# wangqiaoli/geometric_mapping

Hardware: AMD Instinct MI355X
Metric: points/sec full segment+fit, 1M-pt synthetic tunnel frame (higher is better)
Workload: dtype f32; 1 GPU; 1000000-pt synthetic tunnel frame (R=2 m, L=12 m, sigma=0.01), rows resident in HBM; k_regime=fixed-k (~256 neighbours), mode=frames, frames_in_flight=4, GPU_MAX_HW_QUEUES=4, ransac_model=cylinder, H=1024, tau=0.03 (extension), parallelism=framesx1

## Files before the change

geometric_mapping_amd/csrc/k_normals.hip:

```cpp
#include <stdlib.h>
#include <string.h>

#include "gm_internal.hpp"

namespace gm {

typedef float v2f __attribute__((ext_vector_type(2)));

__device__ __forceinline__ v2f pk_mul_rn(v2f a, v2f b)
{
    v2f r;
    r.x = __fmul_rn(a.x, b.x);
    r.y = __fmul_rn(a.y, b.y);
    return r;
}
__device__ __forceinline__ v2f pk_add_rn(v2f a, v2f b)
{
    v2f r;
    r.x = __fadd_rn(a.x, b.x);
    r.y = __fadd_rn(a.y, b.y);
    return r;
}

__device__ __forceinline__ v2f pk_within(v2f d2, v2f neg_big, v2f r2_big)
// ... 391 lines not shown
    uint64_t remaining = __ballot(vox_ok);
    while (remaining) {
        const int leader = (int)__builtin_ctzll(remaining);
        const uint32_t k = __shfl(vkey, leader, kWave);
        const bool mine = vox_ok && vkey == k;
        const uint64_t same = __ballot(mine);
        const unsigned long long ax = wave_total_u64(mine ? fx : 0ull);
        const unsigned long long ay = wave_total_u64(mine ? fy : 0ull);
        const unsigned long long az = wave_total_u64(mine ? fz : 0ull);
        if (lane == leader) {
            VoxCell *cell = vox_table + k;
            atomicAdd(&cell->sx, ax);
            atomicAdd(&cell->sy, ay);
            atomicAdd(&cell->sz, az);
            atomicAdd(&cell->cnt, (uint32_t)__popcll(same));
        }
        remaining &= ~same;
    }
}

struct NormalsArgs {
    const float4 *__restrict__ spts4;
    const uint32_t *__restrict__ skeys;
    const uint2 *__restrict__ tiles;
    DevCounters *__restrict__ ctr;
    GridParams g;
    uint32_t tiles_cap;
    uint32_t tile_seg;
    const uint2 *__restrict__ row_bounds;
    float4 *__restrict__ normals4;
    int32_t *__restrict__ counts;
    VoxDense vd;
    VoxCell *__restrict__ vox_table;
};

constexpr int kValuWaveLdsBytes = 3 * (kWinCap + kWinPad) * 4 + 10 * kWave * 8;
__device__ __forceinline__ void normals_tile_valu(const NormalsArgs &A, unsigned char *lds, const uint2 tile)
{
    const float4 *__restrict__ spts4 = A.spts4;
    const uint32_t *__restrict__ skeys = A.skeys;
    DevCounters *__restrict__ ctr = A.ctr;
    const GridParams &g = A.g;
    const uint2 *__restrict__ row_bounds = A.row_bounds;
    float4 *__restrict__ normals4 = A.normals4;
    int32_t *__restrict__ counts = A.counts;
    const VoxDense &vd = A.vd;
    VoxCell *__restrict__ vox_table = A.vox_table;
    (void)ctr;
    typedef float WinT[3][kWinCap + kWinPad];
    typedef double TotT[10][kWave];
    WinT *win = reinterpret_cast<WinT *>(lds);
    TotT *tot = reinterpret_cast<TotT *>(lds + sizeof(WinT));
    const int lane = lane_id();
    const int w = 0;
    const uint32_t n = ctr->n_cropped;
    {
        const uint32_t qs = tile.x, qn = tile.y & 0xFFu;
#ifdef GM_NORMALS_TIMELINE
        const unsigned long long stat_t0 = wall_clock64();
#endif

        const int ql = lane;
        const bool active = (uint32_t)ql < qn;
        const uint32_t qidx = qs + (active ? (uint32_t)ql : qn - 1u);
        const float4 q = spts4[qidx];
        const uint32_t kl = skeys[qidx];
// ... 434 lines not shown
constexpr int kMdChunk = GM_MDCHUNK;
constexpr int kMdSlots = kMdChunk + 24;
constexpr int kMdOctets = kMdSlots / 8;
constexpr int kMdOctetWords = 33 * 4;
constexpr int kMdWaveLdsBytes = (kMdOctets * kMdOctetWords + 16) * 4;

constexpr int kRowX[3] = {1, 4, 8}, kRowY[3] = {2, 5, 9}, kRowZ[3] = {3, 6, 10}, kRowQ[3] = {11, 7, 12};
constexpr int kRowProd0 = 13;
__device__ __forceinline__ uint32_t md_window_of_base(int b)
{
    return b < 3 ? 0u : ((b == 3 || b == 8) ? 4u : (b == 9 ? 8u : (b == 10 ? 12u : 0u)));
}
__device__ __forceinline__ void md_split3(float a, uint32_t out[3])
{
    const uint32_t ah = __float_as_uint(a) & 0xFFFF0000u;
    const float ra = a - __uint_as_float(ah);
    const uint32_t am = __float_as_uint(ra) & 0xFFFF0000u;
    const float sa = ra - __uint_as_float(am);
    out[0] = ah >> 16; out[1] = am >> 16; out[2] = __float_as_uint(sa) >> 16;
}
__device__ __forceinline__ s4 md_tr_read(const unsigned char *p)
{
    return __builtin_amdgcn_ds_read_tr16_b64_v4i16((__attribute__((address_space(3))) s4 *)p);
}

#ifndef GM_NORMALS_PREFETCH
#define GM_NORMALS_PREFETCH 1
#endif
#ifdef GM_NORMALS_TIMELINE
__device__ unsigned long long gm_tl_buf[3 * 65536];
#endif
#ifdef GM_NORMALS_PHASES
__device__ unsigned long long gm_phase_ticks[16];
#define GM_PH_STAMP(var) const unsigned long long var = __builtin_amdgcn_s_memtime()
#define GM_PH_ADD(slot, expr) do { ph_acc[slot] += (uint32_t)(expr); } while (0)
#else
#define GM_PH_STAMP(var) do {} while (0)
#define GM_PH_ADD(slot, expr) do {} while (0)
#endif

template <bool FINE>
__device__ __forceinline__ void normals_tile_mxd(const NormalsArgs &A, unsigned char *lds, const uint2 tile, uint32_t min_candidates,
                                                 unsigned long long stat_entry = 0ull)
{
    const float4 *__restrict__ spts4 = A.spts4;
    const uint32_t *__restrict__ skeys = A.skeys;
    DevCounters *__restrict__ ctr = A.ctr;
    const GridParams &g = A.g;
    const uint2 *__restrict__ row_bounds = A.row_bounds;
    float4 *__restrict__ normals4 = A.normals4;
    int32_t *__restrict__ counts = A.counts;
    const VoxDense &vd = A.vd;
    VoxCell *__restrict__ vox_table = A.vox_table;
    (void)ctr;
    uint32_t *feat = reinterpret_cast<uint32_t *>(lds);
    int lane = lane_id();
    asm volatile("" : "+v"(lane));
    const uint32_t n = ctr->n_cropped;
    const int qsel = lane & 31, half = lane >> 5;
    const int tq = (lane & 15) >> 2, tp = lane & 3, tr0 = 16 * ((lane >> 4) & 1);
    const uint32_t tr_off = md_window_of_base(8 * half + tq) * 16u +
                            (uint32_t)((tr0 + 4 * tp) >> 3) * (uint32_t)(kMdOctetWords * 4) + (uint32_t)((tr0 + 4 * tp) & 7) * 2u;
    const uint32_t mom_off = (uint32_t)qsel * 16u + 8u * (uint32_t)half;
    {
        const uint32_t qs = tile.x, qn = tile.y & 0xFFu, tile_row = tile.y >> 8;
#ifdef GM_NORMALS_TIMELINE
        const unsigned long long stat_t0 = wall_clock64();
#else
        const unsigned long long stat_t0 = 0ull;
#endif
#ifdef GM_NORMALS_PHASES
        uint32_t ph_acc[8] = {0, 0, 0, 0, 0, 0, 0, 0};
#endif
        GM_PH_STAMP(ph_t0);
        const bool active = (uint32_t)lane < qn;
        const uint32_t qidx = qs + (active ? (uint32_t)lane : qn - 1u);
        const float4 q = spts4[qidx];
        const uint32_t kl = skeys[qidx];
        const uint32_t row = tile_row;
        const int cy = (int)(row % (uint32_t)g.ny), cz = (int)(row / (uint32_t)g.ny);
        const int gD = FINE ? g.D : 1;
        const int side = 2 * gD + 1, nrows_all = side * side;
        int nrows = 0;
        struct LaneRow { int gg, reach; uint32_t nrow; bool ok; uint2 rb; };
        auto lane_row = [&](int row0) -> LaneRow {
            nrows = nrows_all - row0 < 32 ? nrows_all - row0 : 32;
            const int k = FINE ? lane : (lane >> 1);
            const int r = row0 + (k >> 1);
            const int a = (r % side) - gD, b = (r / side) - gD;
            const int yy = cy + a, zz = cz + b;
            LaneRow R;
            R.gg = k & 1;
            R.reach = (k >> 1) < nrows ? (FINE ? (int)g.reach[a < 0 ? -a : a][b < 0 ? -b : b] : g.xreach) : 0;
            R.ok = R.reach > 0 && yy >= 0 && yy < g.ny && zz >= 0 && zz < g.nz;
            R.nrow = R.ok ? (uint32_t)(zz * g.ny + yy) : 0u;
            R.rb = R.ok ? row_bounds[R.nrow] : make_uint2(0u, 0u);
            return R;
        };
        const LaneRow lr0 = lane_row(0);
        const int fxl = (int)(kl - row * (uint32_t)g.nx);
        if (__ballot(active && q.x >= vd.own_lo && q.x < vd.own_hi) == 0) {
            if (active) {
                const float nanv = __builtin_nanf("");
                normals4[__float_as_uint(q.w)] = make_float4(nanv, nanv, nanv, nanv);
                if (counts) counts[__float_as_uint(q.w)] = 0;
            }
            return;
        }
        uint32_t sb = 0, se = 0;
        auto win_begin = [&](int r, int gg) -> uint32_t {
            return FINE ? __builtin_amdgcn_readlane(sb, r * kMxGroups + gg) : __builtin_amdgcn_readlane(sb, 2 * (r * kMxGroups + gg));
        };
        auto win_end = [&](int r, int gg) -> uint32_t {
            return FINE ? __builtin_amdgcn_readlane(se, r * kMxGroups + gg) : __builtin_amdgcn_readlane(sb, 2 * (r * kMxGroups + gg) + 1);
        };
        auto find_windows = [&](const LaneRow &R) {
            sb = 0; se = 0;
            const int gg = R.gg, reach = R.reach;
            const int lo_fx = __shfl(fxl, gg * kMxGroupLanes, kWave);
            const int hi_fx = __shfl(fxl, gg * kMxGroupLanes + kMxGroupLanes - 1, kWave);
            uint32_t key_b = 0, key_e = 0, lo1 = 0, hi1 = 0, row_key0 = 0;
            if (R.ok) {
                const uint32_t rbk = R.nrow * (uint32_t)g.nx;
                const int xa = lo_fx > reach ? lo_fx - reach : 0;
                const int xb = hi_fx + reach < g.nx - 1 ? hi_fx + reach : g.nx - 1;
                key_b = rbk + (uint32_t)xa; key_e = rbk + (uint32_t)xb + 1u;
                lo1 = R.rb.x; hi1 = R.rb.y; row_key0 = rbk;
            }
            if (FINE) {
                uint32_t lo2 = lo1, hi2 = hi1;
                while (lo1 < hi1 || lo2 < hi2) {
                    const uint32_t m1 = (lo1 + hi1) >> 1, m2 = (lo2 + hi2) >> 1;
                    const uint32_t k1 = skeys[m1 < n ? m1 : n - 1u], k2 = skeys[m2 < n ? m2 : n - 1u];
                    if (lo1 < hi1) { if (k1 < key_b) lo1 = m1 + 1u; else hi1 = m1; }
                    if (lo2 < hi2) { if (k2 < key_e) lo2 = m2 + 1u; else hi2 = m2; }
                }
                sb = lo1; se = lo2;
            } else {
                const uint32_t key = (lane & 1) ? key_e : key_b;
#ifndef GM_NORMALS_NO_GUIDED_PROBE
                constexpr uint32_t kGuide = 64;
                if (hi1 - lo1 > 8u * kGuide) {
                    const uint32_t xq = key - row_key0;
                    const uint32_t gpos = lo1 + (uint32_t)((float)xq * (float)(hi1 - lo1) / (float)g.nx);
                    const uint32_t pa0 = gpos > lo1 + kGuide ? gpos - kGuide : lo1;
                    const uint32_t pb0 = gpos + kGuide < hi1 ? gpos + kGuide : hi1 - 1u;
                    const uint32_t ka0 = skeys[pa0], kb0 = skeys[pb0];
                    if (ka0 < key) lo1 = pa0 + 1u; else hi1 = pa0;
                    if (pb0 >= lo1 && pb0 < hi1) { if (kb0 < key) lo1 = pb0 + 1u; else hi1 = pb0; }
                }
#endif
                while (lo1 < hi1) {
                    const uint32_t m1 = (lo1 + hi1) >> 1;
                    if (skeys[m1] < key) lo1 = m1 + 1u; else hi1 = m1;
                }
                sb = lo1;
            }
        };
        find_windows(lr0);
        GM_PH_STAMP(ph_t1);
        GM_PH_ADD(0, ph_t1 - ph_t0);
        bool thin = false;
        if (!FINE) {
            uint32_t wl = 0;
#pragma unroll
            for (int r = 0; r < 9; ++r)
                wl += win_end(r, 0) - win_begin(r, 0);
            thin = wl < min_candidates;
        }
        const int mid = (int)(qn >> 1);
        const float inv_snap = 1.0f / g.snap;
        const float ox = rintf(__uint_as_float(__builtin_amdgcn_readlane(__float_as_uint(q.x), mid)) * inv_snap) * g.snap,
                    oy = rintf(__uint_as_float(__builtin_amdgcn_readlane(__float_as_uint(q.y), mid)) * inv_snap) * g.snap,
                    oz = rintf(__uint_as_float(__builtin_amdgcn_readlane(__float_as_uint(q.z), mid)) * inv_snap) * g.snap;
#ifdef GM_MD_DEBUG
        const float band = g.band;
#endif
        const int ngroups = qn > (uint32_t)kMxGroupLanes ? 2 : 1;
        f32x16 acc[kMxGroups];

#pragma unroll
        for (int gi = 0; gi < kMxGroups; ++gi)
#pragma unroll
            for (int k = 0; k < 16; ++k) acc[gi][k] = 0.f;

        bf16x8 qb[kMxGroups][2];
        float gq[kMxGroups][3];
#pragma unroll
        for (int gi = 0; gi < kMxGroups; ++gi) {
            gq[gi][0] = __shfl(q.x, gi * kMxGroupLanes + qsel, kWave);
            gq[gi][1] = __shfl(q.y, gi * kMxGroupLanes + qsel, kWave);
            gq[gi][2] = __shfl(q.z, gi * kMxGroupLanes + qsel, kWave);
            const float vx = gq[gi][0] - ox, vy = gq[gi][1] - oy, vz = gq[gi][2] - oz;
            const float vv = __fadd_rn(__fadd_rn(__fmul_rn(vx, vx), __fmul_rn(vy, vy)), __fmul_rn(vz, vz));
            uint32_t sv[3], sx[3], sy[3], sz[3];
            const float S = g.dscale;
            md_split3(__fsub_rn(g.r2, vv) * S, sv); md_split3(2.0f * S * vx, sx); md_split3(2.0f * S * vy, sy); md_split3(2.0f * S * vz, sz);
            const uint32_t one = __float_as_uint(-S) >> 16;
            const uint32_t lo0[8] = {sv[0], sv[1], sv[2], sx[0], sx[0], sx[1], sx[2], sy[0]};
            const uint32_t lo1[8] = {sy[0], sy[1], sy[2], sz[0], sz[0], sz[1], sz[2], one};
            const uint32_t hi0[8] = {sx[1], sx[0], one, 0u, sy[1], sy[0], 0u, 0u};
            const uint32_t hi1[8] = {sz[1], sz[0], 0u, 0u, 0u, one, 0u, 0u};
            union { bf16x8 v; uint32_t u[4]; } f0, f1;
#pragma unroll
            for (int j = 0; j < 4; ++j) {
                f0.u[j] = half ? (hi0[2 * j] | (hi0[2 * j + 1] << 16)) : (lo0[2 * j] | (lo0[2 * j + 1] << 16));
                f1.u[j] = half ? (hi1[2 * j] | (hi1[2 * j + 1] << 16)) : (lo1[2 * j] | (lo1[2 * j + 1] << 16));
            }
            qb[gi][0] = f0.v; qb[gi][1] = f1.v;
        }
        auto row_begin = [&](int r) -> uint32_t { return win_begin(r, 0); };
        auto row_end = [&](int r) -> uint32_t { return win_end(r, ngroups - 1); };
        if (thin) {
#if defined(GM_NORMALS_STATS) && !defined(GM_MD_DEBUG)
            if (lane == 0) atomicAdd(&ctr->pad[4], 1u);
#endif
            double tm[10] = {0, 0, 0, 0, 0, 0, 0, 0, 0, 0};
            for (int r = 0; r < 9; ++r) {
                const uint32_t e = row_end(r);
                for (uint32_t i = row_begin(r); i < e; ++i) {
                    const float4 c = spts4[i];
                    const float dx = c.x - q.x, dy = c.y - q.y, dz = c.z - q.z;
                    const float d2 = __fadd_rn(__fadd_rn(__fmul_rn(dx, dx), __fmul_rn(dy, dy)), __fmul_rn(dz, dz));
                    if (d2 < g.r2) {
                        const double ex = dx, ey = dy, ez = dz;
                        tm[0] += 1.0; tm[1] += ex; tm[2] += ey; tm[3] += ez;
                        tm[4] += ex * ex; tm[5] += ex * ey; tm[6] += ex * ez; tm[7] += ey * ey; tm[8] += ey * ez; tm[9] += ez * ez;
                    }
                }
            }
            const bool vox_ok = emit_normal(active, q, tm, vd, normals4, counts, qn, stat_t0);
            if (vd.enabled) voxel_sums(vox_ok, q, vd, vox_table);
            return;
        }
        uint32_t gs = 0, stream_total = 0, nxt_c = 0;
        const int endl = 2 * (ngroups - 1) + 1;
        if (!FINE) {
            const int rl = lane & ~3;
            const uint32_t rb = __shfl(sb, rl, kWave), re = __shfl(sb, rl + endl, kWave);
            const bool rowlane = lane < 36;
            const uint32_t len = rowlane ? re - rb : 0u;
            const uint32_t padded = (len + 7u) & ~7u;
            uint32_t incl = padded;
            incl += (uint32_t)__builtin_amdgcn_update_dpp(0, (int)incl, 0x114 , 0xF, 0xF, true);
            incl += (uint32_t)__builtin_amdgcn_update_dpp(0, (int)incl, 0x118 , 0xF, 0xF, true);
            incl += (uint32_t)__builtin_amdgcn_update_dpp(0, (int)incl, 0x142 , 0xA, 0xF, false);
            incl += (uint32_t)__builtin_amdgcn_update_dpp(0, (int)incl, 0x143 , 0xC, 0xF, false);
            const uint32_t srow = incl - padded;
            const uint32_t s_next = __shfl(incl, 4 * (lane - 40), kWave);
            const uint32_t off_r = __shfl(rb - srow, 4 * (lane - 50), kWave);
            gs = rowlane ? srow + (sb - rb) : ((lane >= 40 && lane < 49) ? s_next : ((lane >= 50 && lane < 59) ? off_r : 0u));
            stream_total = __builtin_amdgcn_readlane(gs, 48);
        }
        GM_PH_STAMP(ph_t2);
        GM_PH_ADD(1, ph_t2 - ph_t1);
        static_assert(kMdChunk == 2 * kWave, "one slot pair per lane and chunk");
        constexpr int kMdPieces = 4;
        int cur_r = 0, row0 = 0;
        uint32_t cur_c = row_begin(0);
        uint32_t n_lo[kMxGroups], n_hi[kMxGroups], n_slots = 0;
        float4 pa = make_float4(0.f, 0.f, 0.f, 0.f), pb = pa;
        uint32_t pidx = qs, pv = 0;
        auto assemble_stream = [&]() {
            n_slots = 0; pv = 0; pidx = qs;
#pragma unroll
            for (int gi = 0; gi < kMxGroups; ++gi) { n_lo[gi] = 0xFFFFFFFFu; n_hi[gi] = 0u; }
// ... 5 lines not shown
            uint32_t r = 0;
#pragma unroll
            for (int k = 0; k < 9; ++k) r += sl0 >= (uint32_t)__builtin_amdgcn_readlane(gs, 40 + k) ? 1u : 0u;
            r = r > 8u ? 8u : r;
            const uint32_t off = __shfl(gs, 50 + (int)r, kWave), lim = __shfl(gs, 4 * (int)r + endl, kWave);
            const bool v0 = sl0 < lim, v1 = sl0 + 1u < lim;
            pidx = v0 ? sl0 + off : qs;
            pv = v0 ? (v1 ? 3u : 1u) : 0u;
            const uint32_t other = __shfl_xor(gs, 1, kWave);
            const uint32_t cb = gs > c0 ? gs : c0, ce = other < c1 ? other : c1;
            const uint64_t m = __ballot((lane & 1) == 0 && lane < 36 && ce > cb);
            const uint32_t cb8 = (cb & ~7u) - c0, ce0 = ce - c0;
#pragma unroll
            for (int gi = 0; gi < kMxGroups; ++gi) {
                if (gi >= ngroups) break;
                const uint64_t mg = m & (gi ? 0x444444444ull : 0x111111111ull);
                if (mg) {
                    n_lo[gi] = __builtin_amdgcn_readlane(cb8, (int)__builtin_ctzll(mg));
                    n_hi[gi] = __builtin_amdgcn_readlane(ce0, 63 - (int)__builtin_clzll(mg));
                }
            }
            pa = spts4[pidx];
            pb = spts4[pidx + (pv >> 1)];
        };
        auto assemble_walk = [&]() {
            n_slots = 0; pv = 0; pidx = qs;
#pragma unroll
            for (int gi = 0; gi < kMxGroups; ++gi) { n_lo[gi] = 0xFFFFFFFFu; n_hi[gi] = 0u; }
            int pieces = 0;
            for (;;) {
                if (cur_r >= nrows) {
                    if (!FINE || row0 + 32 >= nrows_all) break;
                    row0 += 32;
                    find_windows(lane_row(row0));
                    cur_r = 0; cur_c = row_begin(0);
                    continue;
                }
                const uint32_t e = row_end(cur_r);
                if (cur_c >= e) {
                    ++cur_r;
                    if (cur_r < nrows) cur_c = row_begin(cur_r);
                    continue;
                }
                const uint32_t len = e - cur_c, room = (uint32_t)kMdChunk - n_slots;
                const uint32_t take = len < room ? len : room;
#pragma unroll
                for (int gi = 0; gi < kMxGroups; ++gi) {
                    if (gi >= ngroups) break;
                    const uint32_t mb = win_begin(cur_r, gi), me = win_end(cur_r, gi);
                    uint32_t ob = mb > cur_c ? mb - cur_c : 0u, oe = me > cur_c ? me - cur_c : 0u;
                    if (ob > take) ob = take;
                    if (oe > take) oe = take;
                    if (oe > ob) {
                        const uint32_t l = n_slots + (ob & ~7u), h = n_slots + oe;
                        n_lo[gi] = l < n_lo[gi] ? l : n_lo[gi];
                        n_hi[gi] = h > n_hi[gi] ? h : n_hi[gi];
                    }
                }
                {
                    const uint32_t i = 2u * (uint32_t)lane;
                    const bool in = i >= n_slots && i < n_slots + take;
                    pidx = in ? cur_c + (i - n_slots) : pidx;
                    pv = in ? (i + 1u < n_slots + take ? 3u : 1u) : pv;
                }
                n_slots += (take + 7u) & ~7u;
                cur_c += take;
                ++pieces;
// ... 137 lines not shown
                    if (__ballot(amin < g.dband)) {
                        uint32_t gqi = (uint32_t)(gi * kMxGroupLanes + qsel);
                        gqi = qs + (gqi < qn ? gqi : qn - 1u);
                        asm volatile("" : "+v"(gqi));
                        const float4 gqv = spts4[gqi];
#pragma unroll
                        for (int k = 0; k < 16; ++k) {
                            const uint32_t rk = (uint32_t)((k & 3) + 8 * (k >> 2) + 4 * half);
                            const bool need = fabsf(d1[k]) < g.dband;
                            if (__ballot(need)) {
                                if (need) {
                                    const float4 c = spts4[feat[((p + rk) >> 3) * (uint32_t)kMdOctetWords + 31u * 4u + ((p + rk) & 7u)]];
                                    const float dx = c.x - gqv.x, dy = c.y - gqv.y, dz = c.z - gqv.z;
                                    const float d2 = __fadd_rn(__fadd_rn(__fmul_rn(dx, dx), __fmul_rn(dy, dy)), __fmul_rn(dz, dz));
                                    const uint32_t wk = (d2 < g.r2 ? 1u : 0u) * 0x3F80u;
                                    pw[k >> 1] = (k & 1) ? ((pw[k >> 1] & 0x0000FFFFu) | (wk << 16)) : ((pw[k >> 1] & 0xFFFF0000u) | wk);
                                }
                            }
                        }
                    }
                    union { bf16x8 v; uint32_t u[4]; } b0, b1;
#pragma unroll
                    for (int k = 0; k < 4; ++k) { b0.u[k] = pw[k]; b1.u[k] = pw[4 + k]; }
                    acc[gi] = __builtin_amdgcn_mfma_f32_32x32x16_bf16(m0.v, b0.v, acc[gi], 0, 0, 0);
                    acc[gi] = __builtin_amdgcn_mfma_f32_32x32x16_bf16(m1.v, b1.v, acc[gi], 0, 0, 0);
                }
            }
#if !GM_NORMALS_PREFETCH
            assemble();
#endif
            GM_PH_STAMP(ph_c3);
            GM_PH_ADD(4, ph_c3 - ph_c2);
        }
        GM_PH_STAMP(ph_t3);
        int lane_e = lane_id();
        asm volatile("" : "+v"(lane_e));
        const int half_e = lane_e >> 5;
        const bool active_e = (uint32_t)lane_e < qn;
        float own[16], got[16];
#pragma unroll
        for (int k = 0; k < 16; ++k) {
            own[k] = half_e ? acc[1][k] : acc[0][k];
            const float snd = half_e ? acc[0][k] : acc[1][k];
            got[k] = __shfl_xor(snd, 32, kWave);
        }
        auto frow = [&](int rr) -> double {
            const int k = 4 * (rr >> 3) + (rr & 3), hh = (rr >> 2) & 1;
            return (double)((hh == half_e) ? own[k] : got[k]);
        };
        double mom[10];
        mom[0] = frow(0);
        mom[1] = (frow(kRowX[0]) + frow(kRowX[1])) + frow(kRowX[2]);
        mom[2] = (frow(kRowY[0]) + frow(kRowY[1])) + frow(kRowY[2]);
        mom[3] = (frow(kRowZ[0]) + frow(kRowZ[1])) + frow(kRowZ[2]);
#pragma unroll
        for (int m = 0; m < 6; ++m) mom[4 + m] = (frow(kRowProd0 + 3 * m) + frow(kRowProd0 + 3 * m + 1)) + frow(kRowProd0 + 3 * m + 2);

        uint32_t qidx_e = qs + (active_e ? (uint32_t)lane_e : qn - 1u);
        asm volatile("" : "+v"(qidx_e));
        const float4 qe = spts4[qidx_e];
        const bool vox_ok = emit_normal(active_e, qe, mom, vd, normals4, counts, qn, stat_t0, stat_entry);
        if (vd.enabled) voxel_sums(vox_ok, qe, vd, vox_table);
        GM_PH_STAMP(ph_t4);
        GM_PH_ADD(5, ph_t4 - ph_t3);
        GM_PH_ADD(6, ph_t4 - ph_t0);
        GM_PH_ADD(7, 1);
#ifdef GM_NORMALS_PHASES
        if (lane < 8) {
            uint32_t v = 0;
#pragma unroll
            for (int k = 0; k < 8; ++k) v = lane == k ? ph_acc[k] : v;
            atomicAdd(&gm_phase_ticks[lane], (unsigned long long)v);
        }
#endif
    }
}

constexpr int kWaveLdsBytes = (kMxWaveLdsBytes + 15) / 16 * 16;

struct TileList {
    uint32_t n;
    uint32_t pre[kTileClasses];
};
__device__ __forceinline__ TileList tile_list(const NormalsArgs &A)
{
    TileList L;
    uint32_t run = 0;
#pragma unroll
    for (int c = 0; c < kTileClasses; ++c) {
        uint32_t k = A.ctr->n_tiles_c[c][0];
        const uint32_t cap = c + 1 < kTileClasses ? A.tile_seg : A.tiles_cap;
        if (k > cap) k = cap;
        L.pre[c] = run;
        run += k;
    }
    L.n = run;
    return L;
}
__device__ __forceinline__ uint2 tile_at(const NormalsArgs &A, const TileList &L, uint32_t v)
{
    uint32_t c = 0, first = 0;
#pragma unroll
    for (int k = 1; k < kTileClasses; ++k)
        if (v >= L.pre[k]) { c = (uint32_t)k; first = L.pre[k]; }
    return A.tiles[(size_t)c * A.tile_seg + (v - first)];
}

__device__ __forceinline__ uint32_t normals_wave_id(const NormalsArgs &A, uint32_t ntiles)
{
    uint32_t vblock = blockIdx.x;
    const uint32_t nblk = (ntiles + kNrWaves - 1) / kNrWaves;
    if (gridDim.x >= nblk && A.vd.xcd_chunk) {
        if (blockIdx.x >= nblk) return 0xFFFFFFFFu;
        const uint32_t cb = A.vd.xcd_chunk, full = nblk / (8u * cb) * (8u * cb);
        if (blockIdx.x < full) {
            const uint32_t xcd = blockIdx.x % 8u, slot = blockIdx.x / 8u;
            vblock = ((slot / cb) * 8u + xcd) * cb + slot % cb;
        }
    }
    return (uint32_t)__builtin_amdgcn_readfirstlane((int)(vblock * kNrWaves + threadIdx.x / kWave));
}

__global__ __launch_bounds__(kNrThreads, GM_MX_WAVES) void k_normals_m(NormalsArgs A, uint32_t mx_min_candidates)
{
    __shared__ __attribute__((aligned(16))) unsigned char lds[kNrWaves][kWaveLdsBytes];
    const TileList L = tile_list(A);
    const uint32_t ntiles = L.n;
    const uint32_t wave_id = normals_wave_id(A, ntiles), n_waves = gridDim.x * kNrWaves;
    for (uint32_t t = wave_id; t < ntiles; t += n_waves)
        normals_tile_mx(A, lds[threadIdx.x / kWave], tile_at(A, L, t), mx_min_candidates);
}

template <bool FINE>
__global__ __launch_bounds__(kNrThreads, GM_MX_WAVES) void k_normals(NormalsArgs A, uint32_t mx_min_candidates)
{
    __shared__ __attribute__((aligned(16))) unsigned char lds[kNrWaves][(kMdWaveLdsBytes + 15) / 16 * 16];
#ifdef GM_NORMALS_TIMELINE
    unsigned long long stat_entry;
    asm volatile("s_memrealtime %0\n\ts_waitcnt lgkmcnt(0)" : "=s"(stat_entry) : : "memory");
#else
    const unsigned long long stat_entry = 0ull;
#endif
    const TileList L = tile_list(A);
    const uint32_t ntiles = L.n;
    const uint32_t wave_id = normals_wave_id(A, ntiles), n_waves = gridDim.x * kNrWaves;
    if (wave_id >= ntiles) return;
    const int wv = __builtin_amdgcn_readfirstlane((int)(threadIdx.x / kWave));
    {
        uint4 *z = reinterpret_cast<uint4 *>(lds[wv]);
        for (int i = lane_id(); i < kMdWaveLdsBytes / 16; i += kWave) z[i] = make_uint4(0u, 0u, 0u, 0u);
    }
#ifdef GM_NORMALS_TIMELINE
    const uint2 tile_tl = tile_at(A, L, wave_id);
    unsigned long long stat_tile;
    asm volatile("s_memrealtime %0\n\ts_waitcnt lgkmcnt(0)" : "=s"(stat_tile) : "v"(tile_tl.x) : "memory");
    normals_tile_mxd<FINE>(A, lds[wv], tile_tl, mx_min_candidates, stat_entry);
    if (wave_id < 65536u && lane_id() == 0) {
        gm_tl_buf[3 * wave_id + 0] = stat_entry;
        gm_tl_buf[3 * wave_id + 1] = stat_tile;
        gm_tl_buf[3 * wave_id + 2] = (unsigned long long)wall_clock64();
    }
#else
    normals_tile_mxd<FINE>(A, lds[wv], tile_at(A, L, wave_id), mx_min_candidates, stat_entry);
#endif
#ifndef GM_NORMALS_NO_LOOP
    if (ntiles > n_waves && wave_id != 0xFFFFFFFFu)
        for (uint32_t t = wave_id + n_waves; t < ntiles; t += n_waves)
            normals_tile_mxd<FINE>(A, lds[wv], tile_at(A, L, t), mx_min_candidates);
#endif
}

__global__ __launch_bounds__(kNrThreads) void k_normals_valu(NormalsArgs A)
{
    __shared__ __attribute__((aligned(16))) unsigned char lds[kNrWaves][(kValuWaveLdsBytes + 15) / 16 * 16];
    const TileList L = tile_list(A);
    const uint32_t ntiles = L.n;
    const uint32_t wave_id = normals_wave_id(A, ntiles), n_waves = gridDim.x * kNrWaves;
    for (uint32_t t = wave_id; t < ntiles; t += n_waves) normals_tile_valu(A, lds[threadIdx.x / kWave], tile_at(A, L, t));
}

int cell_key_bits(const GridParams &g)
{
    const uint64_t ncell = (uint64_t)g.nx * g.ny * g.nz;
    int bits = 1;
    while ((1ull << bits) < ncell) ++bits;
    return bits;
}

static double inv_below(uint32_t d) { return nextafter(1.0 / (double)(d ? d : 1u), 0.0); }

uint32_t max_tiles(uint32_t n_cap, const GridParams &g)
{
    const uint64_t span = (uint64_t)kTileSpan * (uint64_t)(g.xreach - 1);
    const uint64_t groups = (uint64_t)g.ny * (uint64_t)g.nz * ((uint64_t)g.nx / (span + 1) + 1);
    const uint64_t extra = (groups < n_cap ? groups : n_cap) + n_cap / kTileQ;
    return (uint32_t)(n_cap / kTileQ + extra + 1);
}

void launch_grid_and_normals(const GridParams &g, const VoxDense &vd, Slot &sl, uint32_t n_cap, bool keep_counts,
                             bool scratch_cleared, hipStream_t s)
{
    if (n_cap == 0) return;
    const int where = launch_radix_sort(sl.keys_a, sl.vals_a, sl.keys_b, sl.vals_b, &sl.ctr->n_cropped, n_cap, cell_key_bits(g),
                                        sl, scratch_cleared, s, sl.crop4, sl.spts4);
    uint32_t *skeys = where ? sl.keys_b : sl.keys_a;
    sl.skeys = skeys;
    if (!scratch_cleared) hipMemsetAsync(sl.row_bounds, 0, sizeof(uint2) * (size_t)g.ny * (size_t)g.nz, s);
    {
        ScanState st = next_scan(sl);
        st.status = sl.tile_rec;
        st.ticket = sl.sort.ticket + 1;
        static const char *to = getenv("GM_TILE_ORDER");
        const uint32_t single_class = to ? (to[0] == 'p' ? 1u : 0u) : (sl.pipelined ? 1u : 0u);
        hipLaunchKernelGGL(k_rows_and_tiles, dim3(tile_cutter_blocks(n_cap)), dim3(kTbThreads), 0, s, (const uint32_t *)skeys, sl.ctr,
                           (uint32_t)g.nx, (uint32_t)(kTileSpan * (g.xreach - 1)), inv_below((uint32_t)g.nx),
                           inv_below((uint32_t)(kTileSpan * (g.xreach - 1)) + 1u), sl.row_bounds, (uint32_t)g.ny * (uint32_t)g.nz, sl.tiles,
                           sl.tiles_cap, sl.tile_seg, st, single_class);
    }
    const uint32_t mt = max_tiles(n_cap, g);
    uint32_t nb = (mt + kNrWaves - 1) / kNrWaves;
    {
        const uint32_t usual = (n_cap / 32u + kNrWaves) / kNrWaves;
        if (nb > usual) nb = usual < 64u ? 64u : usual;
    }
    {
        static const char *e = getenv("GM_NORMALS_BLOCKS");
        const uint32_t cap = e ? (uint32_t)atoi(e) : 65536u;
        if (nb > cap) nb = cap;
    }
    static const char *xc = getenv("GM_NORMALS_XCD");
    VoxDense vdx = vd;
    vdx.xcd_chunk = xc ? (uint32_t)atoi(xc) : 32u;
    NormalsArgs na;
    na.spts4 = sl.spts4; na.skeys = skeys; na.tiles = sl.tiles; na.ctr = sl.ctr; na.g = g; na.tiles_cap = sl.tiles_cap; na.tile_seg = sl.tile_seg;
    na.row_bounds = sl.row_bounds; na.normals4 = sl.normals4; na.counts = keep_counts ? sl.counts : (int32_t *)nullptr;
    na.vd = vdx; na.vox_table = sl.vox_table;
    static const char *impl = getenv("GM_NORMALS_IMPL");
    const uint32_t mx_min = !impl ? (uint32_t)kMxMinCandidates : (impl[0] == 'v' ? 0xFFFFFFFFu : (impl[0] == 'm' ? 0u : (uint32_t)kMxMinCandidates));
    if (!sl.capturing) hipEventRecord(sl.ev_k0, s);
    const bool dist_on_mx = !(impl && strchr(impl, '0'));
    if (mx_min == 0xFFFFFFFFu) hipLaunchKernelGGL(k_normals_valu, dim3(nb), dim3(kNrThreads), 0, s, na);
    else if (dist_on_mx) {
        if (g.D > 1) hipLaunchKernelGGL(k_normals<true>, dim3(nb), dim3(kNrThreads), 0, s, na, mx_min);
        else hipLaunchKernelGGL(k_normals<false>, dim3(nb), dim3(kNrThreads), 0, s, na, mx_min);
    }
    else hipLaunchKernelGGL(k_normals_m, dim3(nb), dim3(kNrThreads), 0, s, na, mx_min);
    if (!sl.capturing) hipEventRecord(sl.ev_k1, s);
}

}

#ifdef GM_NORMALS_STATS
extern "C" int gm_debug_counters(gm_ctx *ctx, uint32_t slot, uint32_t *out)
{
    hipDeviceSynchronize();
    gm::DevCounters c;
    const int rc = (int)hipMemcpy(&c, ctx->slots[slot].ctr, sizeof(c), hipMemcpyDeviceToHost);
    memcpy(out, &c, 18 * sizeof(uint32_t));
    out[2] = 0;
    for (int k = 0; k < gm::kTileListClasses; ++k) out[2] += c.n_tiles_c[k][0];
    return rc;
}
#endif

#ifdef GM_NORMALS_TIMELINE
extern "C" int gm_debug_timeline(unsigned long long *out, uint32_t n)
{
    hipDeviceSynchronize();
    if (n > 65536u) n = 65536u;
    return (int)hipMemcpyFromSymbol(out, HIP_SYMBOL(gm::gm_tl_buf), sizeof(unsigned long long) * 3 * (size_t)n);
}
#endif

// ... 19 lines not shown
```

Baseline: 5.303 billion points/s.

## Process tile pairs per wave, overlapping next tile's head loads with epilogue

Each normals wave now handles two consecutive tiles. It issues the second tile's query, key and row-bound loads and its guided-probe search loads while the first tile's epilogue solve and voxel sums run. When both tiles share a grid row, the first tile's window start seeds the second tile's binary search to shrink its range. The block count is halved, which reduces parallelism and occupancy and adds register pressure from holding two tile states. Pairing is on by default for the non-fine MX path and can be disabled with an environment variable.

New measurement: 5.180 billion points/s. 2.3% lower.

```diff
diff --git a/geometric_mapping_amd/csrc/k_normals.hip b/geometric_mapping_amd/csrc/k_normals.hip
--- a/geometric_mapping_amd/csrc/k_normals.hip
+++ b/geometric_mapping_amd/csrc/k_normals.hip
@@ -447,6 +447,7 @@
     int32_t *__restrict__ counts;
     VoxDense vd;
     VoxCell *__restrict__ vox_table;
+    uint32_t pair;
 };
 
 constexpr int kValuWaveLdsBytes = 3 * (kWinCap + kWinPad) * 4 + 10 * kWave * 8;
@@ -947,16 +948,120 @@
 #endif
 #ifdef GM_NORMALS_PHASES
 __device__ unsigned long long gm_phase_ticks[16];
+struct MxdPhases { uint32_t v[10] = {0, 0, 0, 0, 0, 0, 0, 0, 0, 0}; int head = 0; unsigned long long t0 = 0; };
 #define GM_PH_STAMP(var) const unsigned long long var = __builtin_amdgcn_s_memtime()
-#define GM_PH_ADD(slot, expr) do { ph_acc[slot] += (uint32_t)(expr); } while (0)
+#define GM_PH_ADD(slot, expr) do { ph.v[slot] += (uint32_t)(expr); } while (0)
 #else
+struct MxdPhases {};
 #define GM_PH_STAMP(var) do {} while (0)
 #define GM_PH_ADD(slot, expr) do {} while (0)
 #endif
 
+
+struct MxdLaneRow { int gg, reach; uint32_t nrow; bool ok; };
 template <bool FINE>
-__device__ __forceinline__ void normals_tile_mxd(const NormalsArgs &A, unsigned char *lds, const uint2 tile, uint32_t min_candidates,
-                                                 unsigned long long stat_entry = 0ull)
+__device__ __forceinline__ MxdLaneRow mxd_lane_row(const GridParams &g, int lane, uint32_t tile_row, int row0)
+{
+    const int cy = (int)(tile_row % (uint32_t)g.ny), cz = (int)(tile_row / (uint32_t)g.ny);
+    const int gD = FINE ? g.D : 1;
+    const int side = 2 * gD + 1, nrows_all = side * side;
+    const int nrows = nrows_all - row0 < 32 ? nrows_all - row0 : 32;
+    const int k = FINE ? lane : (lane >> 1);
+    const int r = row0 + (k >> 1);
+    const int a = (r % side) - gD, b = (r / side) - gD;
+    const int yy = cy + a, zz = cz + b;
+    MxdLaneRow R;
+    R.gg = k & 1;
+    R.reach = (k >> 1) < nrows ? (FINE ? (int)g.reach[a < 0 ? -a : a][b < 0 ? -b : b] : g.xreach) : 0;
+    R.ok = R.reach > 0 && yy >= 0 && yy < g.ny && zz >= 0 && zz < g.nz;
+    R.nrow = R.ok ? (uint32_t)(zz * g.ny + yy) : 0u;
+    return R;
+}
+
+struct TileHead {
+    uint2 tile;
+    float4 q;
+    uint32_t kl;
+    uint2 rb;
+    uint32_t lo, hi, key, pa, pb, ka, kb;
+    bool guided;
+};
+
+template <bool FINE>
+__device__ __forceinline__ TileHead mxd_head_issue(const NormalsArgs &A, const uint2 tile)
+{
+    int lane = lane_id();
+    asm volatile("" : "+v"(lane));
+    const uint32_t qs = tile.x, qn = tile.y & 0xFFu, tile_row = tile.y >> 8;
+    TileHead H;
+    H.tile = tile;
+    const uint32_t qidx = qs + ((uint32_t)lane < qn ? (uint32_t)lane : qn - 1u);
+    H.q = A.spts4[qidx];
+    H.kl = A.skeys[qidx];
+    const MxdLaneRow R = mxd_lane_row<FINE>(A.g, lane, tile_row, 0);
+    H.rb = A.row_bounds[R.nrow];
+    H.lo = H.hi = H.key = H.pa = H.pb = H.ka = H.kb = 0u;
+    H.guided = false;
+    return H;
+}
+
+constexpr uint32_t kGuide = 64;
+__device__ __forceinline__ void mxd_search_begin(const NormalsArgs &A, TileHead &H, bool seeded, uint32_t seed)
+{
+    int lane = lane_id();
+    asm volatile("" : "+v"(lane));
+    const GridParams &g = A.g;
+    const uint32_t tile_row = H.tile.y >> 8;
+    const MxdLaneRow R = mxd_lane_row<false>(g, lane, tile_row, 0);
+    const int fxl = (int)(H.kl - tile_row * (uint32_t)g.nx);
+    const int lo_fx = __shfl(fxl, R.gg * kMxGroupLanes, kWave);
+    const int hi_fx = __shfl(fxl, R.gg * kMxGroupLanes + kMxGroupLanes - 1, kWave);
+    uint32_t key_b = 0, key_e = 0, lo1 = 0, hi1 = 0, row_key0 = 0;
+    if (R.ok) {
+        const uint32_t rbk = R.nrow * (uint32_t)g.nx;
+        const int xa = lo_fx > R.reach ? lo_fx - R.reach : 0;
+        const int xb = hi_fx + R.reach < g.nx - 1 ? hi_fx + R.reach : g.nx - 1;
+        key_b = rbk + (uint32_t)xa; key_e = rbk + (uint32_t)xb + 1u;
+        lo1 = H.rb.x; hi1 = H.rb.y; row_key0 = rbk;
+    }
+    const uint32_t key = (lane & 1) ? key_e : key_b;
+    const uint32_t row_lo = lo1;
+    if (seeded && R.ok) {
+        const uint32_t s = seed < hi1 ? seed : hi1;
+        lo1 = s > lo1 ? s : lo1;
+    }
+    H.guided = false;
+#ifndef GM_NORMALS_NO_GUIDED_PROBE
+    H.guided = hi1 - lo1 > 8u * kGuide;
+    if (H.guided) {
+        const uint32_t xq = key - row_key0;
+        const uint32_t gpos = row_lo + (uint32_t)((float)xq * (float)(hi1 - row_lo) / (float)g.nx);
+        H.pa = gpos > lo1 + kGuide ? gpos - kGuide : lo1;
+        H.pb = gpos + kGuide < hi1 ? gpos + kGuide : hi1 - 1u;
+        H.ka = A.skeys[H.pa]; H.kb = A.skeys[H.pb];
+    }
+#endif
+    H.lo = lo1; H.hi = hi1; H.key = key;
+}
+__device__ __forceinline__ uint32_t mxd_search_finish(const NormalsArgs &A, const TileHead &H)
+{
+    uint32_t lo1 = H.lo, hi1 = H.hi;
+    const uint32_t key = H.key;
+    if (H.guided) {
+        if (H.ka < key) lo1 = H.pa + 1u; else hi1 = H.pa;
+        if (H.pb >= lo1 && H.pb < hi1) { if (H.kb < key) lo1 = H.pb + 1u; else hi1 = H.pb; }
+    }
+    while (lo1 < hi1) {
+        const uint32_t m1 = (lo1 + hi1) >> 1;
+        if (A.skeys[m1] < key) lo1 = m1 + 1u; else hi1 = m1;
+    }
+    return lo1;
+}
+
+template <bool FINE>
+__device__ __forceinline__ bool mxd_body(const NormalsArgs &A, unsigned char *lds, TileHead &H, bool begun, bool seeded_in,
+                                         uint32_t seed_in, f32x16 (&acc)[kMxGroups], uint32_t min_candidates, bool want_seed,
+                                         uint32_t &seed, MxdPhases &ph)
 {
     const float4 *__restrict__ spts4 = A.spts4;
     const uint32_t *__restrict__ skeys = A.skeys;
@@ -967,7 +1072,8 @@
     int32_t *__restrict__ counts = A.counts;
     const VoxDense &vd = A.vd;
     VoxCell *__restrict__ vox_table = A.vox_table;
-    (void)ctr;
+    (void)ctr; (void)ph;
+    const uint2 tile = H.tile;
     uint32_t *feat = reinterpret_cast<uint32_t *>(lds);
     int lane = lane_id();
     asm volatile("" : "+v"(lane));
@@ -979,48 +1085,21 @@
     const uint32_t mom_off = (uint32_t)qsel * 16u + 8u * (uint32_t)half;
     {
         const uint32_t qs = tile.x, qn = tile.y & 0xFFu, tile_row = tile.y >> 8;
-#ifdef GM_NORMALS_TIMELINE
-        const unsigned long long stat_t0 = wall_clock64();
-#else
         const unsigned long long stat_t0 = 0ull;
-#endif
-#ifdef GM_NORMALS_PHASES
-        uint32_t ph_acc[8] = {0, 0, 0, 0, 0, 0, 0, 0};
-#endif
         GM_PH_STAMP(ph_t0);
         const bool active = (uint32_t)lane < qn;
-        const uint32_t qidx = qs + (active ? (uint32_t)lane : qn - 1u);
-        const float4 q = spts4[qidx];
-        const uint32_t kl = skeys[qidx];
-        const uint32_t row = tile_row;
-        const int cy = (int)(row % (uint32_t)g.ny), cz = (int)(row / (uint32_t)g.ny);
+        const float4 q = H.q;
         const int gD = FINE ? g.D : 1;
         const int side = 2 * gD + 1, nrows_all = side * side;
-        int nrows = 0;
-        struct LaneRow { int gg, reach; uint32_t nrow; bool ok; uint2 rb; };
-        auto lane_row = [&](int row0) -> LaneRow {
-            nrows = nrows_all - row0 < 32 ? nrows_all - row0 : 32;
-            const int k = FINE ? lane : (lane >> 1);
-            const int r = row0 + (k >> 1);
-            const int a = (r % side) - gD, b = (r / side) - gD;
-            const int yy = cy + a, zz = cz + b;
-            LaneRow R;
-            R.gg = k & 1;
-            R.reach = (k >> 1) < nrows ? (FINE ? (int)g.reach[a < 0 ? -a : a][b < 0 ? -b : b] : g.xreach) : 0;
-            R.ok = R.reach > 0 && yy >= 0 && yy < g.ny && zz >= 0 && zz < g.nz;
-            R.nrow = R.ok ? (uint32_t)(zz * g.ny + yy) : 0u;
-            R.rb = R.ok ? row_bounds[R.nrow] : make_uint2(0u, 0u);
-            return R;
-        };
-        const LaneRow lr0 = lane_row(0);
-        const int fxl = (int)(kl - row * (uint32_t)g.nx);
+        int nrows = nrows_all < 32 ? nrows_all : 32;
+        const int fxl = (int)(H.kl - tile_row * (uint32_t)g.nx);
         if (__ballot(active && q.x >= vd.own_lo && q.x < vd.own_hi) == 0) {
             if (active) {
                 const float nanv = __builtin_nanf("");
                 normals4[__float_as_uint(q.w)] = make_float4(nanv, nanv, nanv, nanv);
                 if (counts) counts[__float_as_uint(q.w)] = 0;
             }
-            return;
+            return false;
         }
         uint32_t sb = 0, se = 0;
         auto win_begin = [&](int r, int gg) -> uint32_t {
@@ -1029,52 +1108,41 @@
         auto win_end = [&](int r, int gg) -> uint32_t {
             return FINE ? __builtin_amdgcn_readlane(se, r * kMxGroups + gg) : __builtin_amdgcn_readlane(sb, 2 * (r * kMxGroups + gg) + 1);
         };
-        auto find_windows = [&](const LaneRow &R) {
+        auto find_windows_fine = [&](const MxdLaneRow &R, const uint2 rb) {
             sb = 0; se = 0;
             const int gg = R.gg, reach = R.reach;
             const int lo_fx = __shfl(fxl, gg * kMxGroupLanes, kWave);
             const int hi_fx = __shfl(fxl, gg * kMxGroupLanes + kMxGroupLanes - 1, kWave);
-            uint32_t key_b = 0, key_e = 0, lo1 = 0, hi1 = 0, row_key0 = 0;
+            uint32_t key_b = 0, key_e = 0, lo1 = 0, hi1 = 0;
             if (R.ok) {
                 const uint32_t rbk = R.nrow * (uint32_t)g.nx;
                 const int xa = lo_fx > reach ? lo_fx - reach : 0;
                 const int xb = hi_fx + reach < g.nx - 1 ? hi_fx + reach : g.nx - 1;
                 key_b = rbk + (uint32_t)xa; key_e = rbk + (uint32_t)xb + 1u;
-                lo1 = R.rb.x; hi1 = R.rb.y; row_key0 = rbk;
-            }
-            if (FINE) {
-                uint32_t lo2 = lo1, hi2 = hi1;
-                while (lo1 < hi1 || lo2 < hi2) {
-                    const uint32_t m1 = (lo1 + hi1) >> 1, m2 = (lo2 + hi2) >> 1;
-                    const uint32_t k1 = skeys[m1 < n ? m1 : n - 1u], k2 = skeys[m2 < n ? m2 : n - 1u];
-                    if (lo1 < hi1) { if (k1 < key_b) lo1 = m1 + 1u; else hi1 = m1; }
-                    if (lo2 < hi2) { if (k2 < key_e) lo2 = m2 + 1u; else hi2 = m2; }
-                }
-                sb = lo1; se = lo2;
-            } else {
-                const uint32_t key = (lane & 1) ? key_e : key_b;
-#ifndef GM_NORMALS_NO_GUIDED_PROBE
-                constexpr uint32_t kGuide = 64;
-                if (hi1 - lo1 > 8u * kGuide) {
-                    const uint32_t xq = key - row_key0;
-                    const uint32_t gpos = lo1 + (uint32_t)((float)xq * (float)(hi1 - lo1) / (float)g.nx);
-                    const uint32_t pa0 = gpos > lo1 + kGuide ? gpos - kGuide : lo1;
-                    const uint32_t pb0 = gpos + kGuide < hi1 ? gpos + kGuide : hi1 - 1u;
-                    const uint32_t ka0 = skeys[pa0], kb0 = skeys[pb0];
-                    if (ka0 < key) lo1 = pa0 + 1u; else hi1 = pa0;
-                    if (pb0 >= lo1 && pb0 < hi1) { if (kb0 < key) lo1 = pb0 + 1u; else hi1 = pb0; }
-                }
-#endif
-                while (lo1 < hi1) {
-                    const uint32_t m1 = (lo1 + hi1) >> 1;
-                    if (skeys[m1] < key) lo1 = m1 + 1u; else hi1 = m1;
-                }
-                sb = lo1;
-            }
+                lo1 = rb.x; hi1 = rb.y;
+            }
+            uint32_t lo2 = lo1, hi2 = hi1;
+            while (lo1 < hi1 || lo2 < hi2) {
+                const uint32_t m1 = (lo1 + hi1) >> 1, m2 = (lo2 + hi2) >> 1;
+                const uint32_t k1 = skeys[m1 < n ? m1 : n - 1u], k2 = skeys[m2 < n ? m2 : n - 1u];
+                if (lo1 < hi1) { if (k1 < key_b) lo1 = m1 + 1u; else hi1 = m1; }
+                if (lo2 < hi2) { if (k2 < key_e) lo2 = m2 + 1u; else hi2 = m2; }
+            }
+            sb = lo1; se = lo2;
         };
-        find_windows(lr0);
+        auto next_pass = [&](int row0) {
+            nrows = nrows_all - row0 < 32 ? nrows_all - row0 : 32;
+            const MxdLaneRow R = mxd_lane_row<FINE>(g, lane, tile_row, row0);
+            find_windows_fine(R, R.ok ? row_bounds[R.nrow] : make_uint2(0u, 0u));
+        };
+        if (FINE) {
+            find_windows_fine(mxd_lane_row<FINE>(g, lane, tile_row, 0), H.rb);
+        } else {
+            if (!begun) mxd_search_begin(A, H, seeded_in, seed_in);
+            sb = mxd_search_finish(A, H);
+        }
         GM_PH_STAMP(ph_t1);
-        GM_PH_ADD(0, ph_t1 - ph_t0);
+        GM_PH_ADD(ph.head, ph_t1 - ph_t0);
         bool thin = false;
         if (!FINE) {
             uint32_t wl = 0;
@@ -1092,7 +1160,6 @@
         const float band = g.band;
 #endif
         const int ngroups = qn > (uint32_t)kMxGroupLanes ? 2 : 1;
-        f32x16 acc[kMxGroups];
 
 #pragma unroll
         for (int gi = 0; gi < kMxGroups; ++gi)
@@ -1146,7 +1213,7 @@
             }
             const bool vox_ok = emit_normal(active, q, tm, vd, normals4, counts, qn, stat_t0);
             if (vd.enabled) voxel_sums(vox_ok, q, vd, vox_table);
-            return;
+            return false;
         }
         uint32_t gs = 0, stream_total = 0, nxt_c = 0;
         const int endl = 2 * (ngroups - 1) + 1;
@@ -1218,7 +1285,7 @@
                 if (cur_r >= nrows) {
                     if (!FINE || row0 + 32 >= nrows_all) break;
                     row0 += 32;
-                    find_windows(lane_row(row0));
+                    next_pass(row0);
                     cur_r = 0; cur_c = row_begin(0);
                     continue;
                 }
@@ -1422,48 +1489,140 @@
             GM_PH_STAMP(ph_c3);
             GM_PH_ADD(4, ph_c3 - ph_c2);
         }
+        if (!FINE && want_seed) {
+            int lane_s = lane_id();
+            asm volatile("" : "+v"(lane_s));
+            seed = gs + __shfl(gs, 50 + (lane_s >> 2), kWave);
+        }
         GM_PH_STAMP(ph_t3);
-        int lane_e = lane_id();
-        asm volatile("" : "+v"(lane_e));
-        const int half_e = lane_e >> 5;
-        const bool active_e = (uint32_t)lane_e < qn;
-        float own[16], got[16];
-#pragma unroll
-        for (int k = 0; k < 16; ++k) {
-            own[k] = half_e ? acc[1][k] : acc[0][k];
-            const float snd = half_e ? acc[0][k] : acc[1][k];
-            got[k] = __shfl_xor(snd, 32, kWave);
-        }
-        auto frow = [&](int rr) -> double {
-            const int k = 4 * (rr >> 3) + (rr & 3), hh = (rr >> 2) & 1;
-            return (double)((hh == half_e) ? own[k] : got[k]);
-        };
-        double mom[10];
-        mom[0] = frow(0);
-        mom[1] = (frow(kRowX[0]) + frow(kRowX[1])) + frow(kRowX[2]);
-        mom[2] = (frow(kRowY[0]) + frow(kRowY[1])) + frow(kRowY[2]);
-        mom[3] = (frow(kRowZ[0]) + frow(kRowZ[1])) + frow(kRowZ[2]);
-#pragma unroll
-        for (int m = 0; m < 6; ++m) mom[4 + m] = (frow(kRowProd0 + 3 * m) + frow(kRowProd0 + 3 * m + 1)) + frow(kRowProd0 + 3 * m + 2);
-
-        uint32_t qidx_e = qs + (active_e ? (uint32_t)lane_e : qn - 1u);
-        asm volatile("" : "+v"(qidx_e));
-        const float4 qe = spts4[qidx_e];
-        const bool vox_ok = emit_normal(active_e, qe, mom, vd, normals4, counts, qn, stat_t0, stat_entry);
-        if (vd.enabled) voxel_sums(vox_ok, qe, vd, vox_table);
-        GM_PH_STAMP(ph_t4);
-        GM_PH_ADD(5, ph_t4 - ph_t3);
-        GM_PH_ADD(6, ph_t4 - ph_t0);
-        GM_PH_ADD(7, 1);
+        GM_PH_ADD(6, ph_t3 - ph_t0);
+    }
+    return true;
+}
+
+__device__ __forceinline__ float4 mxd_epilogue_query(const NormalsArgs &A, const uint2 tile)
+{
+    int lane_e = lane_id();
+    asm volatile("" : "+v"(lane_e));
+    const uint32_t qs = tile.x, qn = tile.y & 0xFFu;
+    uint32_t qidx_e = qs + ((uint32_t)lane_e < qn ? (uint32_t)lane_e : qn - 1u);
+    asm volatile("" : "+v"(qidx_e));
+    return A.spts4[qidx_e];
+}
+__device__ __forceinline__ bool mxd_epilogue_solve(const NormalsArgs &A, const uint2 tile, const float4 qe, const f32x16 (&acc)[kMxGroups],
+                                                   MxdPhases &ph)
+{
+    (void)ph;
+    const uint32_t qn = tile.y & 0xFFu;
+    GM_PH_STAMP(ph_t3);
+    int lane_e = lane_id();
+    asm volatile("" : "+v"(lane_e));
+    const int half_e = lane_e >> 5;
+    const bool active_e = (uint32_t)lane_e < qn;
+    float own[16], got[16];
+#pragma unroll
+    for (int k = 0; k < 16; ++k) {
+        own[k] = half_e ? acc[1][k] : acc[0][k];
+        const float snd = half_e ? acc[0][k] : acc[1][k];
+        got[k] = __shfl_xor(snd, 32, kWave);
+    }
+    auto frow = [&](int rr) -> double {
+        const int k = 4 * (rr >> 3) + (rr & 3), hh = (rr >> 2) & 1;
+        return (double)((hh == half_e) ? own[k] : got[k]);
+    };
+    double mom[10];
+    mom[0] = frow(0);
+    mom[1] = (frow(kRowX[0]) + frow(kRowX[1])) + frow(kRowX[2]);
+    mom[2] = (frow(kRowY[0]) + frow(kRowY[1])) + frow(kRowY[2]);
+    mom[3] = (frow(kRowZ[0]) + frow(kRowZ[1])) + frow(kRowZ[2]);
+#pragma unroll
+    for (int m = 0; m < 6; ++m) mom[4 + m] = (frow(kRowProd0 + 3 * m) + frow(kRowProd0 + 3 * m + 1)) + frow(kRowProd0 + 3 * m + 2);
+    const bool vox_ok = emit_normal(active_e, qe, mom, A.vd, A.normals4, A.counts, qn, 0ull, 0ull);
+    GM_PH_STAMP(ph_t4);
+    GM_PH_ADD(5, ph_t4 - ph_t3);
+    GM_PH_ADD(6, ph_t4 - ph_t3);
+    return vox_ok;
+}
+__device__ __forceinline__ void mxd_epilogue_voxels(const NormalsArgs &A, bool vox_ok, const float4 qe, MxdPhases &ph)
+{
+    (void)ph;
+    GM_PH_STAMP(ph_t3);
+    if (A.vd.enabled) voxel_sums(vox_ok, qe, A.vd, A.vox_table);
+    GM_PH_STAMP(ph_t4);
+    GM_PH_ADD(5, ph_t4 - ph_t3);
+    GM_PH_ADD(6, ph_t4 - ph_t3);
+    GM_PH_ADD(7, 1);
 #ifdef GM_NORMALS_PHASES
-        if (lane < 8) {
-            uint32_t v = 0;
-#pragma unroll
-            for (int k = 0; k < 8; ++k) v = lane == k ? ph_acc[k] : v;
-            atomicAdd(&gm_phase_ticks[lane], (unsigned long long)v);
-        }
-#endif
-    }
+    if (ph.head) ph.v[9] += 1u;
+    const int lane_p = lane_id();
+    if (lane_p < 10) {
+        uint32_t v = 0;
+#pragma unroll
+        for (int k = 0; k < 10; ++k) v = lane_p == k ? ph.v[k] : v;
+        atomicAdd(&gm_phase_ticks[lane_p], (unsigned long long)v);
+    }
+#endif
+}
+
+template <bool FINE>
+__device__ __forceinline__ void normals_tile_mxd(const NormalsArgs &A, unsigned char *lds, const uint2 tile, uint32_t min_candidates)
+{
+    MxdPhases ph;
+    GM_PH_STAMP(ph_h0);
+    TileHead H = mxd_head_issue<FINE>(A, tile);
+    GM_PH_STAMP(ph_h1);
+    GM_PH_ADD(0, ph_h1 - ph_h0);
+    GM_PH_ADD(6, ph_h1 - ph_h0);
+    f32x16 acc[kMxGroups];
+    uint32_t seed = 0;
+    if (!mxd_body<FINE>(A, lds, H, false, false, 0u, acc, min_candidates, false, seed, ph)) return;
+    const float4 qe = mxd_epilogue_query(A, tile);
+    const bool vox_ok = mxd_epilogue_solve(A, tile, qe, acc, ph);
+    mxd_epilogue_voxels(A, vox_ok, qe, ph);
+}
+
+template <bool FINE>
+__device__ __forceinline__ void normals_pair_mxd(const NormalsArgs &A, unsigned char *lds, const uint2 tile_a, const uint2 tile_b,
+                                                 bool has_b, uint32_t min_candidates)
+{
+    MxdPhases ph_a, ph_b;
+#ifdef GM_NORMALS_PHASES
+    ph_b.head = 8;
+#endif
+    const bool same_row = has_b && (tile_b.y >> 8) == (tile_a.y >> 8) && tile_b.x > tile_a.x;
+    f32x16 acc[kMxGroups];
+    uint32_t seed = 0;
+    bool open_a;
+    {
+        MxdPhases &ph = ph_a;
+        (void)ph;
+        GM_PH_STAMP(ph_h0);
+        TileHead HA = mxd_head_issue<FINE>(A, tile_a);
+        GM_PH_STAMP(ph_h1);
+        GM_PH_ADD(0, ph_h1 - ph_h0);
+        GM_PH_ADD(6, ph_h1 - ph_h0);
+        open_a = mxd_body<FINE>(A, lds, HA, false, false, 0u, acc, min_candidates, !FINE && same_row, seed, ph_a);
+    }
+    const bool seeded = !FINE && same_row && open_a;
+    const float4 qe = mxd_epilogue_query(A, tile_a);
+    MxdPhases &ph = ph_b;
+    (void)ph;
+    GM_PH_STAMP(ph_b0);
+    TileHead HB = mxd_head_issue<FINE>(A, tile_b);
+    GM_PH_STAMP(ph_b1);
+    bool vox_ok = false;
+    if (open_a) vox_ok = mxd_epilogue_solve(A, tile_a, qe, acc, ph_a);
+    GM_PH_STAMP(ph_b2);
+    if (!FINE) mxd_search_begin(A, HB, seeded, seed);
+    GM_PH_STAMP(ph_b3);
+    GM_PH_ADD(8, (ph_b1 - ph_b0) + (ph_b3 - ph_b2));
+    GM_PH_ADD(6, (ph_b1 - ph_b0) + (ph_b3 - ph_b2));
+    if (open_a) mxd_epilogue_voxels(A, vox_ok, qe, ph_a);
+    if (!has_b) return;
+    if (!mxd_body<FINE>(A, lds, HB, true, false, 0u, acc, min_candidates, false, seed, ph_b)) return;
+    const float4 qb = mxd_epilogue_query(A, tile_b);
+    const bool vox_b = mxd_epilogue_solve(A, tile_b, qb, acc, ph_b);
+    mxd_epilogue_voxels(A, vox_b, qb, ph_b);
 }
 
 constexpr int kWaveLdsBytes = (kMxWaveLdsBytes + 15) / 16 * 16;
@@ -1496,13 +1655,13 @@
     return A.tiles[(size_t)c * A.tile_seg + (v - first)];
 }
 
-__device__ __forceinline__ uint32_t normals_wave_id(const NormalsArgs &A, uint32_t ntiles)
+__device__ __forceinline__ uint32_t normals_wave_id(const NormalsArgs &A, uint32_t nwork, uint32_t per = 1u)
 {
     uint32_t vblock = blockIdx.x;
-    const uint32_t nblk = (ntiles + kNrWaves - 1) / kNrWaves;
+    const uint32_t nblk = (nwork + kNrWaves - 1) / kNrWaves;
     if (gridDim.x >= nblk && A.vd.xcd_chunk) {
         if (blockIdx.x >= nblk) return 0xFFFFFFFFu;
-        const uint32_t cb = A.vd.xcd_chunk, full = nblk / (8u * cb) * (8u * cb);
+        const uint32_t cb = A.vd.xcd_chunk >= per ? A.vd.xcd_chunk / per : 1u, full = nblk / (8u * cb) * (8u * cb);
         if (blockIdx.x < full) {
             const uint32_t xcd = blockIdx.x % 8u, slot = blockIdx.x / 8u;
             vblock = ((slot / cb) * 8u + xcd) * cb + slot % cb;
@@ -1533,30 +1692,41 @@
 #endif
     const TileList L = tile_list(A);
     const uint32_t ntiles = L.n;
-    const uint32_t wave_id = normals_wave_id(A, ntiles), n_waves = gridDim.x * kNrWaves;
-    if (wave_id >= ntiles) return;
+    const uint32_t per = A.pair ? 2u : 1u;
+    const uint32_t nwork = (ntiles + per - 1u) / per;
+    const uint32_t wave_id = normals_wave_id(A, nwork, per), n_waves = gridDim.x * kNrWaves;
+    if (wave_id >= nwork) return;
     const int wv = __builtin_amdgcn_readfirstlane((int)(threadIdx.x / kWave));
     {
         uint4 *z = reinterpret_cast<uint4 *>(lds[wv]);
         for (int i = lane_id(); i < kMdWaveLdsBytes / 16; i += kWave) z[i] = make_uint4(0u, 0u, 0u, 0u);
     }
+    const uint32_t ta = wave_id * per;
+    const bool has_b = A.pair && ta + 1u < ntiles;
+    const uint2 tile_a = tile_at(A, L, ta), tile_b = tile_at(A, L, has_b ? ta + 1u : ta);
 #ifdef GM_NORMALS_TIMELINE
-    const uint2 tile_tl = tile_at(A, L, wave_id);
     unsigned long long stat_tile;
-    asm volatile("s_memrealtime %0\n\ts_waitcnt lgkmcnt(0)" : "=s"(stat_tile) : "v"(tile_tl.x) : "memory");
-    normals_tile_mxd<FINE>(A, lds[wv], tile_tl, mx_min_candidates, stat_entry);
+    asm volatile("s_memrealtime %0\n\ts_waitcnt lgkmcnt(0)" : "=s"(stat_tile) : "v"(tile_a.x) : "memory");
+#endif
+    if (A.pair && !FINE) normals_pair_mxd<FINE>(A, lds[wv], tile_a, tile_b, has_b, mx_min_candidates);
+    else {
+        normals_tile_mxd<FINE>(A, lds[wv], tile_a, mx_min_candidates);
+        if (has_b) normals_tile_mxd<FINE>(A, lds[wv], tile_b, mx_min_candidates);
+    }
+#ifdef GM_NORMALS_TIMELINE
     if (wave_id < 65536u && lane_id() == 0) {
         gm_tl_buf[3 * wave_id + 0] = stat_entry;
         gm_tl_buf[3 * wave_id + 1] = stat_tile;
         gm_tl_buf[3 * wave_id + 2] = (unsigned long long)wall_clock64();
     }
-#else
-    normals_tile_mxd<FINE>(A, lds[wv], tile_at(A, L, wave_id), mx_min_candidates, stat_entry);
-#endif
+#endif
+    (void)stat_entry;
 #ifndef GM_NORMALS_NO_LOOP
-    if (ntiles > n_waves && wave_id != 0xFFFFFFFFu)
-        for (uint32_t t = wave_id + n_waves; t < ntiles; t += n_waves)
-            normals_tile_mxd<FINE>(A, lds[wv], tile_at(A, L, t), mx_min_candidates);
+    if (nwork > n_waves && wave_id != 0xFFFFFFFFu)
+        for (uint32_t u = wave_id + n_waves, k = 0; u < nwork && u * per + k < ntiles;) {
+            normals_tile_mxd<FINE>(A, lds[wv], tile_at(A, L, u * per + k), mx_min_candidates);
+            if (++k == per) { k = 0; u += n_waves; }
+        }
 #endif
 }
 
@@ -1613,6 +1783,12 @@
         const uint32_t usual = (n_cap / 32u + kNrWaves) / kNrWaves;
         if (nb > usual) nb = usual < 64u ? 64u : usual;
     }
+    static const char *impl = getenv("GM_NORMALS_IMPL");
+    const uint32_t mx_min = !impl ? (uint32_t)kMxMinCandidates : (impl[0] == 'v' ? 0xFFFFFFFFu : (impl[0] == 'm' ? 0u : (uint32_t)kMxMinCandidates));
+    const bool dist_on_mx = mx_min != 0xFFFFFFFFu && !(impl && strchr(impl, '0'));
+    static const char *pe = getenv("GM_NORMALS_PAIR");
+    const uint32_t pair = dist_on_mx && !(pe && pe[0] == '0') ? 1u : 0u;
+    if (pair) nb = (nb + 1u) / 2u;
     {
         static const char *e = getenv("GM_NORMALS_BLOCKS");
         const uint32_t cap = e ? (uint32_t)atoi(e) : 65536u;
@@ -1624,11 +1800,8 @@
     NormalsArgs na;
     na.spts4 = sl.spts4; na.skeys = skeys; na.tiles = sl.tiles; na.ctr = sl.ctr; na.g = g; na.tiles_cap = sl.tiles_cap; na.tile_seg = sl.tile_seg;
     na.row_bounds = sl.row_bounds; na.normals4 = sl.normals4; na.counts = keep_counts ? sl.counts : (int32_t *)nullptr;
-    na.vd = vdx; na.vox_table = sl.vox_table;
-    static const char *impl = getenv("GM_NORMALS_IMPL");
-    const uint32_t mx_min = !impl ? (uint32_t)kMxMinCandidates : (impl[0] == 'v' ? 0xFFFFFFFFu : (impl[0] == 'm' ? 0u : (uint32_t)kMxMinCandidates));
+    na.vd = vdx; na.vox_table = sl.vox_table; na.pair = pair;
     if (!sl.capturing) hipEventRecord(sl.ev_k0, s);
-    const bool dist_on_mx = !(impl && strchr(impl, '0'));
     if (mx_min == 0xFFFFFFFFu) hipLaunchKernelGGL(k_normals_valu, dim3(nb), dim3(kNrThreads), 0, s, na);
     else if (dist_on_mx) {
         if (g.D > 1) hipLaunchKernelGGL(k_normals<true>, dim3(nb), dim3(kNrThreads), 0, s, na, mx_min);
```
